# shangzhouye/stereo-visual-slam

Hardware: AMD Instinct MI355X
Metric: stereo keyframes/sec (ORB+match+tri+local-BA), KITTI-00 1241x376 (higher is better)
Workload: dtype u8+f64

## Files before the change

stereo-visual-slam_amd/csrc/api.hip:

```cpp
#include <stdarg.h>
#include <stdlib.h>

#include <algorithm>
#include <cmath>
#include <cfloat>
#include <vector>

#include "se3_device.h"
#include "vslam_internal.h"

#include <mutex>

namespace vslam {

static thread_local char g_err[512] = "";
void set_error(const char* fmt, ...) {
    va_list ap;
    va_start(ap, fmt);
    vsnprintf(g_err, sizeof(g_err), fmt, ap);
    va_end(ap);
}

struct Prof {
    struct Rec { const char* name; int launches; hipEvent_t e0, e1; };
    bool on = false;
    std::vector<Rec> recs, open;
    std::vector<hipEvent_t> pool;
    hipEvent_t get() {
        if (!pool.empty()) { hipEvent_t e = pool.back(); pool.pop_back(); return e; }
        hipEvent_t e = nullptr;
        (void)hipEventCreate(&e);
        return e;
    }
};
static thread_local Prof* g_prof = nullptr;
static hipEvent_t g_prof_origin[16] = {nullptr};
static std::mutex g_prof_origin_mu;
Prof* prof_current() { return g_prof; }
void prof_set_current(Prof* p) { g_prof = p; }
void prof_begin(hipStream_t s, const char* name, int launches) {
    Prof* p = g_prof;
    if (!p || !p->on) return;
    Prof::Rec r{name, launches, p->get(), p->get()};
    (void)hipEventRecord(r.e0, s);
    p->open.push_back(r);
}
void prof_end(hipStream_t s) {
    Prof* p = g_prof;
    if (!p || !p->on || p->open.empty()) return;
    Prof::Rec r = p->open.back();
    p->open.pop_back();
    (void)hipEventRecord(r.e1, s);
    p->recs.push_back(r);
}
#define VS_ENTER(c)                                                                         \
    do {                                                                                    \
        VS_HIP(hipSetDevice((c)->device));                                                  \
        prof_set_current(((c)->prof && (c)->prof->on) ? (c)->prof : nullptr);               \
    } while (0)

int DevBuf::reserve(size_t need, hipStream_t stream) {
    if (bytes >= need) return VSLAM_OK;
    VS_HIP(hipStreamSynchronize(stream));
    release();
    const size_t want = std::max(need, min_bytes);
    if (hipMalloc((void**)&p, want) != hipSuccess) { p = nullptr; set_error("%s hipMalloc(%zu) failed", name, want); return VSLAM_ERR_HIP; }
    bytes = want; *acct += want;
    return VSLAM_OK;
}
void DevBuf::release() {
    if (p) { (void)hipFree(p); *acct -= bytes; }
    p = nullptr; bytes = 0;
}

struct Arena : Layout {
    struct Upload { void* d; const void* h; size_t bytes; };
    std::vector<Upload> uploads;
    explicit Arena(uint8_t* b = nullptr) : Layout(b) {}
    template <typename T> T* in(const T* h, size_t n) { T* d = take<T>(n); if (base) uploads.push_back({d, h, n * sizeof(T)}); return d; }
};
template <typename F>
static int arena_stage(Ctx* c, F&& layout) {
    Arena a;
    if (int rc = carve(c->stage, c->stream, a, layout)) return rc;
    for (const Arena::Upload& u : a.uploads) VS_HIP(hipMemcpyAsync(u.d, u.h, u.bytes, hipMemcpyHostToDevice, c->stream));
    return VSLAM_OK;
}

static CamParams cam_of(const Ctx* c) {
    CamParams cam;
    cam.fx = c->p.cam[0]; cam.fy = c->p.cam[1]; cam.cx = c->p.cam[2]; cam.cy = c->p.cam[3]; cam.b = c->p.cam[4];
    cam.dmin = c->p.depth_min; cam.dmax = c->p.depth_max; cam.drel = c->p.depth_reliable; cam.row_tol = c->p.stereo_row_tol;
    return cam;
}

template <typename T>
static int dev_alloc(Ctx* c, T** p, size_t n) {
    VS_HIP(hipMalloc((void**)p, n * sizeof(T)));
    c->dev_bytes += n * sizeof(T);
    return VSLAM_OK;
}

struct TuneKey { const char* name; const char* env; int Tuning::*field; int lo, hi; };
static const TuneKey kTuneKeys[] = {
    {"orb_fuse_min", "VSLAM_ORB_FUSE_MIN", &Tuning::orb_fuse_min, 0, 1 << 30},
    {"sgbm_fuse_min", "VSLAM_SGBM_FUSE_MIN", &Tuning::sgbm_fuse_min, 0, 1 << 30},
    {"sgbm_fwd_min", "VSLAM_SGBM_FWD_MIN", &Tuning::sgbm_fwd_min, 0, 1 << 30},
    {"sgbm_fw_rows", "VSLAM_SGBM_FW_ROWS", &Tuning::sgbm_fw_rows, 32, 64},
    {"pose_only_window", "VSLAM_POSE_ONLY_WINDOW", &Tuning::pose_only_window, 0, 1},
    {"ba_resident", "VSLAM_BA_RESIDENT", &Tuning::ba_resident, 0, 1},
    {"pnp_window", "VSLAM_PNP_WINDOW", &Tuning::pnp_window, 0, 1},
    {"ba_adaptive", "VSLAM_BA_ADAPTIVE", &Tuning::ba_adaptive, 0, 1},
    {"ba_lanes", "VSLAM_BA_LANES", &Tuning::ba_lanes, 256, 512},
    {"track_rule", "VSLAM_TRACK_RULE", &Tuning::track_rule, 0, 1},
};
static int tune_set(Tuning& t, const TuneKey& k, long v) {
    if (v == -1) { t.*(k.field) = -1; return VSLAM_OK; }
    if (v < k.lo || v > k.hi || (k.field == &Tuning::sgbm_fw_rows && v != 32 && v != 64) || (k.field == &Tuning::ba_lanes && v != 256 && v != 512)) {
        set_error("tuning value %s = %ld out of range (%d..%d%s, or -1 = default)", k.name, v, k.lo, k.hi, k.field == &Tuning::sgbm_fw_rows ? ", 32 or 64" : "");
        return VSLAM_ERR_ARG;
    }
    t.*(k.field) = (int)v;
    return VSLAM_OK;
}
static int tune_from_env(Tuning& t) {
    for (const TuneKey& k : kTuneKeys) {
        const char* e = getenv(k.env);
        if (!e || !*e) continue;
        char* end = nullptr;
        const long v = strtol(e, &end, 10);
        if (end == e || *end != 0) { set_error("environment variable %s = \"%s\" is not an integer", k.env, e); return VSLAM_ERR_ARG; }
        int rc = tune_set(t, k, v);
        if (rc) return rc;
    }
    return VSLAM_OK;
}

static int orb_status_check(Ctx* c, int B) {
    std::vector<int32_t> st(B);
    VS_HIP(hipMemcpyAsync(st.data(), c->orb.d_status, sizeof(int32_t) * B, hipMemcpyDeviceToHost, c->stream));
    VS_HIP(hipStreamSynchronize(c->stream));
    for (int b = 0; b < B; ++b)
        if (st[b]) { set_error("ORB capacity exceeded on image %d (status bits 0x%x)", b, st[b]); return VSLAM_ERR_CAPACITY; }
    return VSLAM_OK;
}

constexpr int kOrbFuseMinDefault = 96;
static int orb_fuse_min(const Ctx* c) { return c->tune.orb_fuse_min >= 0 ? c->tune.orb_fuse_min : kOrbFuseMinDefault; }

static int orb_pipeline(Ctx* c, const uint8_t* d_imgs, size_t img_bytes, int pitch, int B, int anms_num, int regroup, bool describe,
                        vslam_keypoint* d_kps, uint8_t* d_desc, int32_t* d_count) {
    if (B <= 0) return VSLAM_OK;
    if (B > c->p.max_batch) { set_error("batch %d exceeds context max_batch %d", B, c->p.max_batch); return VSLAM_ERR_ARG; }
    int rc;
    const bool fused = describe && B >= orb_fuse_min(c);
    if (fused) {
        if ((rc = launch_orb_pyrblur(c->plan, c->tab, d_imgs, img_bytes, pitch, B, c->orb.d_pyr, c->orb.d_blur, c->p.fast_threshold, c->orb.d_corners,
                                     c->orb.d_corner_cnt, c->orb.d_status, c->stream))) return rc;
    } else {
        if ((rc = launch_orb_pyramid(c->plan, c->tab, d_imgs, img_bytes, pitch, B, c->orb.d_pyr, c->stream))) return rc;
        if ((rc = launch_orb_fast(c->plan, d_imgs, img_bytes, pitch, B, c->orb.d_pyr, c->p.fast_threshold, c->orb.d_corners,
                                  c->orb.d_corner_cnt, c->orb.d_status, c->stream))) return rc;
    }
    if ((rc = launch_orb_select(c->plan, d_imgs, img_bytes, pitch, B, c->orb.d_pyr, c->orb.d_corners, c->orb.d_corner_cnt, c->orb.d_sel,
                                c->orb.d_sel_cnt, c->orb.d_status, c->stream))) return rc;
    if ((rc = launch_orb_anms(c->plan, B, c->orb.d_sel, c->orb.d_sel_cnt, c->plan.sel_cap, anms_num, regroup, d_kps, nullptr, c->orb.d_order, c->p.kp_capacity,
                              d_count, c->orb.d_status, c->orb.d_rad, c->stream))) return rc;
    if ((rc = launch_orb_orient(c->plan, d_imgs, img_bytes, pitch, B, c->orb.d_pyr, d_kps, c->orb.d_cs, c->orb.d_order, c->p.kp_capacity, d_count, c->stream))) return rc;
    if (describe) {
        if (!fused && (rc = launch_orb_blur(c->plan, d_imgs, img_bytes, pitch, B, c->orb.d_pyr, c->orb.d_blur, c->stream))) return rc;
        if ((rc = launch_orb_describe(c->plan, d_imgs, img_bytes, pitch, B, c->orb.d_pyr, c->orb.d_blur, d_kps, c->orb.d_cs, c->orb.d_order, c->p.kp_capacity, d_count,
                                      d_desc, c->stream))) return rc;
    }
    if (getenv("VSLAM_ORB_PROFILE")) orb_debug_dump(c->stream);
    return VSLAM_OK;
}

static int check_img(Ctx* c, const void* img, int w, int h, int stride) {
    if (!c || !img) { set_error("null context or image"); return VSLAM_ERR_ARG; }
    if (w != c->p.img_w || h != c->p.img_h || stride < w) { set_error("image %dx%d (stride %d) does not match the context's %dx%d", w, h, stride, c->p.img_w, c->p.img_h); return VSLAM_ERR_ARG; }
    return VSLAM_OK;
}

}

using namespace vslam;

extern "C" {

void vslam_default_params(vslam_params* p) {
    if (!p) return;
    memset(p, 0, sizeof(*p));
    p->img_w = 1241; p->img_h = 376; p->max_batch = 1;
    p->orb_nfeatures = 3000; p->anms_num = 500; p->fast_threshold = 20; p->kp_capacity = 4096;
    p->cam[0] = 718.856; p->cam[1] = 718.856; p->cam[2] = 607.1928; p->cam[3] = 185.2157; p->cam[4] = 0.573;
    p->depth_min = 10; p->depth_max = 400; p->depth_reliable = 40;
    p->match_ratio = 2.0; p->match_gap_thr = 30.0; p->huber_delta = 5.991; p->pnp_reproj_thr = 4.0; p->stereo_row_tol = 2.0;
    p->struct_size = (int32_t)sizeof(vslam_params); p->abi_version = VSLAM_ABI_VERSION;
}

const char* vslam_last_error(void) { return g_err; }
const char* vslam_version(void) { return "vslam_hip 0.3 (gfx950, ABI 3)"; }
int vslam_abi_version(void) { return VSLAM_ABI_VERSION; }
const char* vslam_kernel_names(void) {
    return "orb_resize_kernel orb_pyrblur_kernel orb_fast_kernel orb_select_kernel orb_anms_kernel orb_orient_kernel orb_blur_kernel orb_describe_kernel "
           "match_train_nearest_kernel match_finalize_kernel sgbm_prefilter_kernel sgbm_down_kernel sgbm_forward_kernel sgbm_hsum_kernel sgbm_vsum_kernel sgbm_path_kernel "
           "sgbm_wta_kernel sgbm_lrcheck_kernel sgbm_median3_kernel sgbm_ccl_rows_kernel sgbm_ccl_union_kernel sgbm_ccl_count_kernel "
           "sgbm_ccl_apply_kernel sgbm_ccl_kernels triangulate_kernel find3d_disparity_kernel gather_uv_kernel build_pnp_inputs_kernel lm_window_kernel pose_only_wave_kernel "
           "lm_window_kernel<pnp> pnp_wave_kernel pnp_inlier_kernel pnp_epnp_kernels epnp_front_kernel epnp_jacobi_kernel epnp_back_kernel pnp_count_inliers_kernel hbm_copy_probe_kernel "
           "pnp_ransac_subsets_kernel pnp_ransac_count_kernel pnp_ransac_select_kernel "
           "build_windows_kernels track_init_kernel track_pose_chain_kernel track_link_kernel track_chain_kernel window_count_kernel window_scan_kernel window_rank_kernel window_emit_kernel "
           "track_ends_kernel kf_band_kernel kf_set_kernel kf_sliding_kernel kf_gate_kernel map_pnp_inputs_kernels track_map_inputs_kernel "
           "match_train_nearest_sel_kernel track_features_kernel";
}

int vslam_create(const vslam_params* p, int device, void* stream, vslam_ctx** out) {
    if (!p || !out) { set_error("null argument"); return VSLAM_ERR_ARG; }
    *out = nullptr;
    if (p->struct_size != (int32_t)sizeof(vslam_params) || p->abi_version != VSLAM_ABI_VERSION) {
        set_error("vslam_params from a different ABI (struct_size %d / abi_version %d, library has %d / %d): rebuild the caller against include/vslam_hip.h and "
                  "fill the struct with vslam_default_params", p->struct_size, p->abi_version, (int)sizeof(vslam_params), VSLAM_ABI_VERSION);
        return VSLAM_ERR_ARG;
    }
    int ndev = 0;
    if (hipGetDeviceCount(&ndev) != hipSuccess || ndev <= 0) { set_error("no HIP device visible (libvslam_hip has no CPU path)"); return VSLAM_ERR_NO_DEVICE; }
    if (device < 0 || device >= ndev) { set_error("device %d out of range (0..%d)", device, ndev - 1); return VSLAM_ERR_ARG; }
    if (p->max_batch <= 0 || p->kp_capacity < 64 || p->kp_capacity > kMaxRows || p->orb_nfeatures <= 0) { set_error("bad params (max_batch>0, 64<=kp_capacity<=%d)", kMaxRows); return VSLAM_ERR_ARG; }
    VS_HIP(hipSetDevice(device));
    Ctx* c = new Ctx();
    c->p = *p; c->device = device;
    c->lm.tune = &c->tune;
    { int rc_t = tune_from_env(c->tune); if (rc_t) { delete c; return rc_t; } }
    if (stream) { c->stream = (hipStream_t)stream; c->own_stream = false; }
    else {
        if (hipStreamCreateWithFlags(&c->stream, hipStreamNonBlocking) != hipSuccess) { set_error("hipStreamCreate failed"); delete c; return VSLAM_ERR_HIP; }
        c->own_stream = true;
    }
    if (getenv("VSLAM_ORB_PROFILE")) orb_debug_enable();
    int rc = orb_plan_init(&c->plan, p->img_w, p->img_h, p->orb_nfeatures, p->kp_capacity);
    if (rc == VSLAM_OK) { rc = orb_tables_init(&c->plan, &c->tab); c->dev_bytes += c->tab.bytes; }
    const size_t B = (size_t)p->max_batch;
    if (rc == VSLAM_OK) rc = dev_alloc(c, &c->orb.d_pyr, B * c->plan.pyr_bytes);
    if (rc == VSLAM_OK) rc = dev_alloc(c, &c->orb.d_corners, B * c->plan.corner_total);
    if (rc == VSLAM_OK) rc = dev_alloc(c, &c->orb.d_corner_cnt, B * kNLevels);
    if (rc == VSLAM_OK) rc = dev_alloc(c, &c->orb.d_sel, B * kNLevels * c->plan.sel_cap);
    if (rc == VSLAM_OK) rc = dev_alloc(c, &c->orb.d_sel_cnt, B * kNLevels);
    if (rc == VSLAM_OK) rc = dev_alloc(c, &c->orb.d_status, B);
    if (rc == VSLAM_OK) rc = dev_alloc(c, &c->orb.d_blur, B * c->plan.blur_bytes);
    if (rc == VSLAM_OK) rc = dev_alloc(c, &c->orb.d_cs, B * (size_t)p->kp_capacity);
    if (rc == VSLAM_OK) rc = dev_alloc(c, &c->orb.d_order, B * (size_t)p->kp_capacity);
    if (rc == VSLAM_OK) rc = dev_alloc(c, &c->orb.d_rad, B * (size_t)kMaxRows);
    if (rc == VSLAM_OK) rc = dev_alloc(c, &c->match.d_train_best, B * kMaxRows);
    if (rc != VSLAM_OK) { vslam_destroy(reinterpret_cast<vslam_ctx*>(c)); return rc; }
    *out = reinterpret_cast<vslam_ctx*>(c);
    return VSLAM_OK;
// ... 1046 lines not shown
```

stereo-visual-slam_amd/csrc/orb_kernels.hip:

```cpp
#include "vslam_internal.h"

#include <math.h>

#include <vector>

#include "orb_pattern.inc"

namespace vslam {

constexpr int kBlurTileH = 64;

__device__ __constant__ signed char c_pattern[256 * 4];

__device__ long long* g_orb_dbg = nullptr;
constexpr int kDbgRows = 8192;
#define OPH_INIT() long long* dbg__ = g_orb_dbg ? g_orb_dbg + 64 * (size_t)((blockIdx.x + 977u * blockIdx.y) % kDbgRows) : nullptr; long long tph__ = dbg__ ? clock64() : 0
#define OPH_ON() (dbg__ != nullptr)
#define OPH(slot) do { if (dbg__ && threadIdx.x == 0) { const long long t1__ = clock64(); dbg__[(slot) & 63] += t1__ - tph__; tph__ = t1__; } } while (0)
static long long* g_orb_dbg_host = nullptr;
void orb_debug_enable() {
    if (g_orb_dbg_host) return;
    hipMalloc((void**)&g_orb_dbg_host, sizeof(long long) * 64 * kDbgRows);
    hipMemset(g_orb_dbg_host, 0, sizeof(long long) * 64 * kDbgRows);
    hipMemcpyToSymbol(HIP_SYMBOL(g_orb_dbg), &g_orb_dbg_host, sizeof(g_orb_dbg_host));
}
void orb_debug_dump(hipStream_t stream) {
    if (!g_orb_dbg_host) return;
    hipStreamSynchronize(stream);
    static long long hall[64 * kDbgRows];
    hipMemcpy(hall, g_orb_dbg_host, sizeof(hall), hipMemcpyDeviceToHost);
    hipMemset(g_orb_dbg_host, 0, sizeof(hall));
    long long h[64] = {0};
    for (int r = 0; r < kDbgRows; ++r) for (int i = 0; i < 64; ++i) h[i] += hall[64 * r + i];
    static const char* names[64] = {"sel: hist+cut", "sel: harris", "sel: radix select", "sel: compact+sort", "sel: angle+out", nullptr, nullptr, nullptr,
                                    "desc: patch load", "desc: row blur", "desc: col blur", "desc: sincos+tests", nullptr, nullptr, nullptr, nullptr,
                                    "fast: tile load", "fast: corner test", "fast: score", "fast: nms+append", nullptr, nullptr, nullptr, nullptr,
                                    "anms: gather+sort", "anms: radii", "anms: radius sort", "anms: compact+regroup+out", nullptr, nullptr, nullptr, nullptr,
                                    "pyrfast: tile load", "pyrfast: resize", "pyrfast: blur", "pyrfast: edge columns", "pyrfast: pre-test", "pyrfast: queue pushes", "pyrfast: scores",
                                    "pyrfast: flush + barrier", "pyrfast: nms", "pyrfast: output"};
    for (int i = 0; i < 64; ++i) if (names[i] && h[i]) fprintf(stderr, "  [orb profile] %-28s %14lld block-cycles (sum over blocks)\n", names[i], h[i]);
}
static bool g_pattern_uploaded[16] = {false};

constexpr int kStCornerOverflow = 1, kStCandOverflow = 2, kStSelOverflow = 4, kStAnmsOverflow = 8, kStOutOverflow = 16;

__device__ inline int reflect101(int p, int len) {
    if (len == 1) return 0;
    while (p < 0 || p >= len) p = p < 0 ? -p : 2 * (len - 1) - p;
    return p;
}

struct LevelView {
    const uint8_t* ptr;
    int w, h, pitch;
};

struct LevelTable {
    int w[kNLevels], h[kNLevels], pitch[kNLevels], pyr_off[kNLevels];
    float scale[kNLevels];
    int nfeat[kNLevels];
    int corner_cap[kNLevels], corner_off[kNLevels];
    int tiles_x[kNLevels], tile_off[kNLevels + 1];
};

__device__ inline LevelView level_view(const LevelTable& T, int l, const uint8_t* img, int pitch0, const uint8_t* pyr) {
    LevelView v;
    v.w = T.w[l]; v.h = T.h[l];
    if (l == 0) { v.ptr = img; v.pitch = pitch0; }
    else { v.ptr = pyr + T.pyr_off[l]; v.pitch = T.pitch[l]; }
    return v;
}

__device__ inline uint4 shl_bytes_128(uint4 v, int s) {
    for (int t = 0; t < (s >> 2); ++t) { v.w = v.z; v.z = v.y; v.y = v.x; v.x = 0; }
    const uint32_t b = (uint32_t)s & 3u;
    if (b) {
        v.w = __builtin_amdgcn_alignbyte(v.w, v.z, 4u - b); v.z = __builtin_amdgcn_alignbyte(v.z, v.y, 4u - b);
        v.y = __builtin_amdgcn_alignbyte(v.y, v.x, 4u - b); v.x <<= 8u * b;
    }
    return v;
}
__device__ inline uint4 shr_bytes_128(uint4 v, int s) {
    for (int t = 0; t < (s >> 2); ++t) { v.x = v.y; v.y = v.z; v.z = v.w; v.w = 0; }
    const uint32_t b = (uint32_t)s & 3u;
    if (b) {
        v.x = __builtin_amdgcn_alignbyte(v.y, v.x, b); v.y = __builtin_amdgcn_alignbyte(v.z, v.y, b);
// ... 1543 lines not shown
            keep = v > s[-1] && v > s[1] && v > s[-kPfScPitch - 1] && v > s[-kPfScPitch] && v > s[-kPfScPitch + 1] && v > s[kPfScPitch - 1] &&
                   v > s[kPfScPitch] && v > s[kPfScPitch + 1];
            rec = (uint32_t)(ox + c - 4) | (uint32_t)(oy + R - 4) << 12 | (uint32_t)v << 24;
        }
        const unsigned long long bal = __ballot(keep);
        if (bal) {
            int base = 0;
            if (lane == 0) base = atomicAdd(&s_ocount, __popcll(bal));
            base = __builtin_amdgcn_readfirstlane(base);
            if (keep) outq[base + mbcnt64(bal)] = rec;
        }
    };
    if (!s_dense) {
        const int nc = s_ccount;
        for (int q = 64 * wave; q < nc; q += NT) nms_emit(q + lane < nc, q + lane < nc ? s_cq[q + lane] : 0);
    } else {
        for (int i = threadIdx.x; i < 64 * kBlurTileH; i += NT) {
            const int r = i >> 6, d = i & 63;
            uint32_t m = reinterpret_cast<const uint32_t*>(sc + (r + 1) * kPfScPitch)[1 + d];
            if (r <= vy_lo || r >= vy_hi) m = 0;
#pragma unroll 1
            for (int k = 0; k < 4; ++k) {
                const int tcx = 4 * d + k;
                const bool is = ((m >> (8 * k)) & 0xFFu) != 0 && tcx > vx_lo && tcx < vx_hi;
                if (__ballot(is)) nms_emit(is, (r + 4) << 9 | (tcx + 4));
            }
        }
    }
    __syncthreads();
    OPH(40);
    const int no = s_ocount;
    if (no > 0) {
        if (threadIdx.x == 0) s_obase = atomicAdd(a.corner_cnt + b * kNLevels, no);
        __syncthreads();
        uint32_t* corners = a.corners + (size_t)b * a.corner_img_stride;
        const int cap = a.corner_cap, base = s_obase;
        for (int q = threadIdx.x; q < no; q += NT) {
            if (base + q < cap) corners[base + q] = outq[q];
            else atomicOr(&a.status[b], kStCornerOverflow);
        }
    }
    OPH(41);
}

int launch_orb_pyrblur(const OrbPlan& plan, const OrbTables& tab, const uint8_t* d_imgs, size_t img_bytes, int pitch, int B, uint8_t* d_pyr,
                       uint8_t* d_blur, int fast_thr, uint32_t* d_corners, int32_t* d_corner_cnt, int32_t* d_status, hipStream_t stream) {
    if (d_corners) {
        VS_HIP(hipMemsetAsync(d_corner_cnt, 0, sizeof(int32_t) * B * kNLevels, stream));
        VS_HIP(hipMemsetAsync(d_status, 0, sizeof(int32_t) * B, stream));
    }
    ProfScope prof__(stream, "orb_pyrblur_kernel", kNLevels);
    for (int l = 0; l < kNLevels; ++l) {
        const OrbLevel& S = plan.lv[l];
        PyrBlurArgs a;
        memset(&a, 0, sizeof(a));
        a.src_base = l == 0 ? d_imgs : d_pyr + S.pyr_off;
        a.src_img_stride = l == 0 ? img_bytes : (size_t)plan.pyr_bytes;
        a.spitch = l == 0 ? pitch : ((S.w + 63) & ~63);
        a.sw = S.w; a.sh = S.h;
        a.blur_base = d_blur + plan.blur_off[l]; a.blur_img_stride = (size_t)plan.blur_bytes; a.bpitch = (S.w + 63) & ~63;
        a.tiles_x = (S.w + kBlurTileW - 1) / kBlurTileW;
        const int tiles_y = (S.h + kBlurTileH - 1) / kBlurTileH;
        if (l + 1 < kNLevels) {
            const OrbLevel& D = plan.lv[l + 1];
            a.dst_base = d_pyr + D.pyr_off; a.dst_img_stride = (size_t)plan.pyr_bytes; a.dpitch = (D.w + 63) & ~63; a.dw = D.w; a.dh = D.h;
            a.xofs = tab.d_xofs + tab.x_off[l + 1]; a.ialpha = tab.d_ialpha + 2 * tab.x_off[l + 1];
            a.yofs = tab.d_yofs + tab.y_off[l + 1]; a.ibeta = tab.d_ibeta + 2 * tab.y_off[l + 1];
            a.tile_dx = tab.d_tile_dx + tab.tdx_off[l]; a.tile_dy = tab.d_tile_dy + tab.tdy_off[l];
        }
        if (d_corners) {
            a.corners = d_corners + S.corner_off; a.corner_img_stride = (size_t)plan.corner_total; a.corner_cap = S.corner_cap;
            a.corner_cnt = d_corner_cnt + l; a.status = d_status; a.thr = fast_thr; a.level = l;
        }
        hipLaunchKernelGGL(orb_pyrblur_kernel<kPfWaves>, dim3(a.tiles_x * tiles_y, B), dim3(64 * kPfWaves), 0, stream, a);
    }
    VS_HIP(hipGetLastError());
    return VSLAM_OK;
}

constexpr int kDescWaves = 4;
constexpr int kDescR = 19, kDescRows = 2 * kDescR + 1, kDescPitch = 40;

constexpr int kDescBlocksPerImage = 48;
constexpr int kDescPatchIters = (kDescRows * (kDescPitch / 4) + 63) / 64;
__global__ __launch_bounds__(kDescWaves * 64) void orb_describe_kernel(BlurTable T, LevelTable LT, const uint8_t* __restrict__ d_imgs,
                                                                      size_t img_bytes, int pitch0, const uint8_t* __restrict__ d_pyr,
                                                                      size_t pyr_bytes, const uint8_t* __restrict__ d_blur, size_t blur_bytes,
                                                                      const vslam_keypoint* __restrict__ d_kps, const float2* __restrict__ d_cs,
                                                                      const int32_t* __restrict__ d_order, int kp_capacity,
                                                                      const int32_t* __restrict__ d_count, uint8_t* __restrict__ d_desc, int nb, int B) {
    int b, bx;
    if (!xcd_image_block(nb, B, b, bx)) return;
    const int wave = __builtin_amdgcn_readfirstlane(threadIdx.x >> 6), lane = threadIdx.x & 63;
    const int nwaves = nb * kDescWaves;
    const int n = min(d_count[b], kp_capacity);
    const int i0 = bx * kDescWaves + wave;
    if (i0 >= n) return;
    int slots;
    {
        const int i = i0 + lane * nwaves;
        slots = i < n ? (d_order ? min(max(d_order[(size_t)b * kp_capacity + i], 0), n - 1) : i) : -1;
    }
    const int nvisit = min((n - i0 + nwaves - 1) / nwaves, 64);
    int visit = 0;
    int j = __builtin_amdgcn_readlane(slots, 0);
    const vslam_keypoint* kps = d_kps + (size_t)b * kp_capacity;
    const float2* css = d_cs + (size_t)b * kp_capacity;
    __shared__ __attribute__((aligned(16))) uint8_t patch[kDescWaves][kDescRows * kDescPitch];
    uint8_t* pl = patch[wave];
    float px0[4], py0[4], px1[4], py1[4];
#pragma unroll
    for (int k = 0; k < 4; ++k) {
        const signed char* q = &c_pattern[(4 * lane + k) * 4];
        px0[k] = (float)q[0]; py0[k] = (float)q[1]; px1[k] = (float)q[2]; py1[k] = (float)q[3];
    }
    int prow[kDescPatchIters], pcol[kDescPatchIters];
#pragma unroll
    for (int it = 0; it < kDescPatchIters; ++it) {
        const int i = lane + 64 * it;
        prow[it] = i / (kDescPitch / 4); pcol[it] = 4 * (i - prow[it] * (kDescPitch / 4));
    }
    struct Geo { int cx, cy, l, W, H, bpitch; bool inside; const uint8_t* blur; };
    auto geometry = [&](const vslam_keypoint& kp) -> Geo {
        Geo g;
        g.l = __builtin_amdgcn_readfirstlane(min(max(kp.octave, 0), kNLevels - 1));
        g.W = T.w[g.l]; g.H = T.h[g.l]; g.bpitch = T.pitch[g.l];
        g.blur = d_blur + (size_t)b * blur_bytes + T.blur_off[g.l];
        const float inv_scale = __fdiv_rn(1.f, LT.scale[g.l]);
        g.cx = __builtin_amdgcn_readfirstlane(__float2int_rn(__fmul_rn(kp.x, inv_scale)));
        g.cy = __builtin_amdgcn_readfirstlane(__float2int_rn(__fmul_rn(kp.y, inv_scale)));
        g.inside = g.cx - kDescR >= 0 && g.cx + kDescR + 1 < g.W && g.cy - kDescR >= 0 && g.cy + kDescR < g.H;
        return g;
    };
    auto patch_fetch = [&](const Geo& g, uint32_t (&pv)[kDescPatchIters]) {
        if (!g.inside) return;
        const uint8_t* org = g.blur + (size_t)(g.cy - kDescR) * g.bpitch + (g.cx - kDescR);
#pragma unroll
        for (int it = 0; it < kDescPatchIters; ++it)
            if (prow[it] < kDescRows) __builtin_memcpy(&pv[it], org + (__umul24((uint32_t)prow[it], (uint32_t)g.bpitch) + (uint32_t)pcol[it]), 4);
    };
    vslam_keypoint kp = kps[j];
    float2 cs = css[j];
    Geo g = geometry(kp);
    uint32_t pv[kDescPatchIters];
    patch_fetch(g, pv);
    auto slot_of = [&](int v) -> int { return v < nvisit ? __builtin_amdgcn_readlane(slots, v) : -1; };
    int j1 = slot_of(1);
    vslam_keypoint kp1 = kps[max(j1, 0)];
    float2 cs1 = css[max(j1, 0)];
    for (;;) {
        if (g.inside) {
#pragma unroll
            for (int it = 0; it < kDescPatchIters; ++it)
                if (prow[it] < kDescRows) *reinterpret_cast<uint32_t*>(pl + prow[it] * kDescPitch + pcol[it]) = pv[it];
        }
        const Geo g1 = geometry(kp1);
        uint32_t pv1[kDescPatchIters];
        if (j1 >= 0) patch_fetch(g1, pv1);
        const int j2 = slot_of(visit + 2);
        const vslam_keypoint kp2 = kps[max(j2, 0)];
        const float2 cs2 = css[max(j2, 0)];
        __builtin_amdgcn_wave_barrier();
        const float ca = cs.x, sa = cs.y;
        int nib = 0;
        if (g.inside) {
#pragma unroll
            for (int k = 0; k < 4; ++k) {
                const int ix0 = __float2int_rn(__fsub_rn(__fmul_rn(px0[k], ca), __fmul_rn(py0[k], sa)));
                const int iy0 = __float2int_rn(__fadd_rn(__fmul_rn(px0[k], sa), __fmul_rn(py0[k], ca)));
                const int ix1 = __float2int_rn(__fsub_rn(__fmul_rn(px1[k], ca), __fmul_rn(py1[k], sa)));
                const int iy1 = __float2int_rn(__fadd_rn(__fmul_rn(px1[k], sa), __fmul_rn(py1[k], ca)));
                const int t0 = pl[(iy0 + kDescR) * kDescPitch + ix0 + kDescR], t1 = pl[(iy1 + kDescR) * kDescPitch + ix1 + kDescR];
                nib |= (t0 < t1) << k;
            }
        } else {
            const uint8_t* rawp = g.l == 0 ? d_imgs + (size_t)b * img_bytes : d_pyr + (size_t)b * pyr_bytes + T.pyr_off[g.l];
            const int rpitch = g.l == 0 ? pitch0 : T.pitch[g.l];
            auto sample = [&](int ix, int iy) -> int {
                const int x = g.cx + ix, y = g.cy + iy;
                if (x >= 0 && x < g.W && y >= 0 && y < g.H) return g.blur[(size_t)y * g.bpitch + x];
                return rawp[(size_t)reflect101(y, g.H) * rpitch + reflect101(x, g.W)];
            };
#pragma unroll
            for (int k = 0; k < 4; ++k) {
                const int ix0 = __float2int_rn(__fsub_rn(__fmul_rn(px0[k], ca), __fmul_rn(py0[k], sa)));
                const int iy0 = __float2int_rn(__fadd_rn(__fmul_rn(px0[k], sa), __fmul_rn(py0[k], ca)));
                const int ix1 = __float2int_rn(__fsub_rn(__fmul_rn(px1[k], ca), __fmul_rn(py1[k], sa)));
                const int iy1 = __float2int_rn(__fadd_rn(__fmul_rn(px1[k], sa), __fmul_rn(py1[k], ca)));
                nib |= (sample(ix0, iy0) < sample(ix1, iy1)) << k;
            }
        }
        const int hi = __shfl_down(nib, 1);
        if ((lane & 1) == 0) d_desc[((size_t)b * kp_capacity + j) * 32 + (lane >> 1)] = (uint8_t)(nib | (hi << 4));
        if (j1 < 0) break;
        __builtin_amdgcn_wave_barrier();
        ++visit;
        j = j1; j1 = j2; g = g1; cs = cs1; kp1 = kp2; cs1 = cs2;
#pragma unroll
        for (int it = 0; it < kDescPatchIters; ++it) pv[it] = pv1[it];
    }
}

int launch_orb_describe(const OrbPlan& plan, const uint8_t* d_imgs, size_t img_bytes, int pitch, int B, const uint8_t* d_pyr,
                        const uint8_t* d_blur, const vslam_keypoint* d_kps, const float2* d_cs, const int32_t* d_order, int kp_capacity, const int32_t* d_count,
                        uint8_t* d_desc, hipStream_t stream) {
    BlurTable T;
    fill_blur_table(plan, &T);
    LevelTable LT;
    fill_level_table(plan, &LT);
    const int max_kp = min(kp_capacity, kMaxRows);
    const int blocks = min(kDescBlocksPerImage, (max_kp + kDescWaves - 1) / kDescWaves);
    ProfScope prof__(stream, "orb_describe_kernel");
    hipLaunchKernelGGL(orb_describe_kernel, dim3(blocks * ((B + 7) / 8 * 8)), dim3(kDescWaves * 64), 0, stream, T, LT, d_imgs,
                       img_bytes, pitch, d_pyr, (size_t)plan.pyr_bytes, d_blur, (size_t)plan.blur_bytes, d_kps, d_cs, d_order, kp_capacity, d_count, d_desc, blocks, B);
    VS_HIP(hipGetLastError());
    return VSLAM_OK;
}

}
```

stereo-visual-slam_amd/csrc/vslam_internal.h:

```cpp
#pragma once
#include <hip/hip_runtime.h>
#include <stdint.h>
#include <stdio.h>
#include <string.h>

#include "../../include/vslam_hip.h"

namespace vslam {

void set_error(const char* fmt, ...);

#define VS_HIP(call)                                                                              \
    do {                                                                                          \
        hipError_t e__ = (call);                                                                  \
        if (e__ != hipSuccess) {                                                                  \
            ::vslam::set_error("%s:%d %s -> %s", __FILE__, __LINE__, #call, hipGetErrorString(e__)); \
            return VSLAM_ERR_HIP;                                                                 \
        }                                                                                         \
    } while (0)

struct Prof;
Prof* prof_current();
void prof_set_current(Prof* p);
void prof_begin(hipStream_t s, const char* name, int launches);
// ... 37 lines not shown
template <typename F>
int carve(DevBuf& buf, hipStream_t stream, F&& layout) { Layout a; return carve(buf, stream, a, layout); }

constexpr int kWave = 64;
constexpr int kNLevels = VSLAM_ORB_NLEVELS;
constexpr int kEdge = 31;
constexpr int kMaxRows = 4096;

struct OrbLevel {
    int w, h;
    float scale;
    int nfeat;
    int pyr_off;
    int corner_cap;
    int corner_off;
    int tiles_x, tiles_y, tile_off;
    int tab_off;
};

struct OrbPlan {
    OrbLevel lv[kNLevels];
    int w, h;
    int pyr_bytes;
    int corner_total;
    int total_tiles;
    int sel_cap;
    int blur_off[kNLevels];
    int blur_bytes;
};

struct Ctx;

struct OrbTables {
    int* d_xofs;
    short* d_ialpha;
    int* d_yofs;
    short* d_ibeta;
    int x_off[kNLevels], y_off[kNLevels];
    int* d_tile_dx;
    int* d_tile_dy;
    int tdx_off[kNLevels], tdy_off[kNLevels];
    size_t bytes;
};

void orb_debug_enable();
void orb_debug_dump(hipStream_t stream);
int orb_plan_init(OrbPlan* plan, int w, int h, int nfeatures, int kp_capacity);
int orb_tables_init(const OrbPlan* plan, OrbTables* t);
void orb_tables_free(OrbTables* t);

struct OrbBuffers {
    uint8_t* d_pyr;
    uint32_t* d_corners;
    int32_t* d_corner_cnt;
    vslam_keypoint* d_sel;
    int32_t* d_sel_cnt;
    int32_t* d_status;
    vslam_keypoint* d_det;
    uint8_t* d_blur;
    float2* d_cs;
    int32_t* d_order;
    double* d_rad;
};

int launch_orb_pyramid(const OrbPlan& plan, const OrbTables& tab, const uint8_t* d_imgs, size_t img_bytes, int pitch,
                       int B, uint8_t* d_pyr, hipStream_t stream);
int launch_orb_pyrblur(const OrbPlan& plan, const OrbTables& tab, const uint8_t* d_imgs, size_t img_bytes, int pitch, int B, uint8_t* d_pyr,
                       uint8_t* d_blur, int fast_thr, uint32_t* d_corners, int32_t* d_corner_cnt, int32_t* d_status, hipStream_t stream);
int launch_orb_fast(const OrbPlan& plan, const uint8_t* d_imgs, size_t img_bytes, int pitch, int B, const uint8_t* d_pyr,
                    int fast_thr, uint32_t* d_corners, int32_t* d_corner_cnt, int32_t* d_status, hipStream_t stream);
int launch_orb_select(const OrbPlan& plan, const uint8_t* d_imgs, size_t img_bytes, int pitch, int B, const uint8_t* d_pyr,
                      const uint32_t* d_corners, const int32_t* d_corner_cnt, vslam_keypoint* d_sel, int32_t* d_sel_cnt,
                      int32_t* d_status, hipStream_t stream);
int launch_orb_anms(const OrbPlan& plan, int B, const vslam_keypoint* d_sel, const int32_t* d_sel_cnt, int sel_cap,
                    int anms_num, int regroup, vslam_keypoint* d_kps, float2* d_cs, int32_t* d_order, int kp_capacity, int32_t* d_count, int32_t* d_status,
                    double* d_rad, hipStream_t stream);
int launch_anms_flat(int B, const vslam_keypoint* d_in, const int32_t* d_nin, int in_capacity, int anms_num, int regroup,
                     int img_w, int img_h, vslam_keypoint* d_kps, float2* d_cs, int32_t* d_order, int kp_capacity, int32_t* d_count, int32_t* d_status,
                     double* d_rad, hipStream_t stream);
int launch_orb_blur(const OrbPlan& plan, const uint8_t* d_imgs, size_t img_bytes, int pitch, int B, const uint8_t* d_pyr, uint8_t* d_blur,
                    hipStream_t stream);
int launch_orb_orient(const OrbPlan& plan, const uint8_t* d_imgs, size_t img_bytes, int pitch, int B, const uint8_t* d_pyr, vslam_keypoint* d_kps,
                      float2* d_cs, const int32_t* d_order, int kp_capacity, const int32_t* d_count, hipStream_t stream);
int launch_orb_describe(const OrbPlan& plan, const uint8_t* d_imgs, size_t img_bytes, int pitch, int B, const uint8_t* d_pyr,
                        const uint8_t* d_blur, const vslam_keypoint* d_kps, const float2* d_cs, const int32_t* d_order, int kp_capacity, const int32_t* d_count,
                        uint8_t* d_desc, hipStream_t stream);

struct MatchBuffers {
    uint32_t* d_train_best;
};
int launch_match(const uint8_t* d_q, size_t q_stride, const int32_t* d_nq, const uint8_t* d_t, size_t t_stride,
                 const int32_t* d_nt, const double* d_gap, int gate, double ratio, double gap_thr, int B, int max_rows,
                 uint32_t* d_train_best, vslam_dmatch* d_out, int out_capacity, int32_t* d_nout, hipStream_t stream,
                 const int32_t* d_qsel = nullptr, int sel_cap = 0, const int32_t* d_nqsel = nullptr);

struct CamParams { double fx, fy, cx, cy, b, dmin, dmax, drel, row_tol; };
int launch_find3d_disparity(const vslam_keypoint* d_kps, int n, const float* d_disp, int w, int h, int dstride,
                            const double* d_T, CamParams cam, float* d_xyz, uint8_t* d_valid, uint8_t* d_rel, hipStream_t stream);
int launch_find3d_disparity_batch(const vslam_keypoint* d_kps, const int32_t* d_n, int kp_capacity, int B, const float* d_disp, int w, int h,
                                  const double* d_T, CamParams cam, float* d_xyz, uint8_t* d_valid, uint8_t* d_rel, hipStream_t stream);
int launch_triangulate(const float* d_uvL, const float* d_uvR, const int32_t* d_n, int capacity, int B, const double* d_T,
                       CamParams cam, float* d_xyz, uint8_t* d_valid, uint8_t* d_rel, hipStream_t stream);
int launch_build_pnp_inputs(const vslam_dmatch* d_m, const int32_t* d_nm, int match_capacity, const vslam_dmatch* d_lr,
                            const int32_t* d_nlr, int lr_capacity, const float* d_xyz_lr, const uint8_t* d_valid_lr,
                            const vslam_keypoint* d_kpsT, int kp_capacity, int B, int32_t* d_kp2lr, float* d_xyz_out, float* d_uv_out,
                            int32_t* d_nout, int out_capacity, hipStream_t stream);
int launch_gather_uv(const vslam_keypoint* d_kpsQ, const vslam_keypoint* d_kpsT, int kp_capacity, const vslam_dmatch* d_m,
                     const int32_t* d_nm, int match_capacity, int B, float* d_uvQ, float* d_uvT, hipStream_t stream);

int launch_hbm_copy_probe(const void* src, void* dst, size_t bytes, int variant, hipStream_t stream);
int hbm_copy_probe_variants();
const char* hbm_copy_probe_name(int variant);

struct LmWindowArgs {
    int n_windows, n_kf;
    const int32_t* n_kf_w;
    const int32_t* lm_off;
    const int32_t* edge_off;
    double* T;
    float* xyz;
    const uint8_t* reliable;
    uint8_t* lm_inlier;
    const int32_t* kf_idx;
    const int32_t* lm_idx;
    const float* uv;
    double* chi2;
    vslam_lm_stats* stats;
    double* P;
    double* Ptrial;
    double* Hll;
    double* bl;
    double* Dinv;
    double* lin;
    int32_t* lm_ptr;
    int32_t* kf_ptr;
    int32_t* kf_edges;
    int32_t* pair_ptr;
    int32_t* pair_hits;
    int32_t hit_capacity_per_edge;
    double K[4];
    double huber_delta;
    double* chi2_thr;
    size_t total_lm, total_edge;
};
struct Tuning {
    int orb_fuse_min = -1;
    int sgbm_fuse_min = -1;
    int sgbm_fwd_min = -1;
    int sgbm_fw_rows = -1;
    int pose_only_window = -1;
    int pnp_window = -1;
    int ba_lanes = -1;
    int ba_resident = -1;
    int track_rule = -1;
    int ba_adaptive = -1;
};
constexpr int kSgbmTicketPools = 8;
constexpr int kSgbmErrorWord = kSgbmTicketPools;
int launch_sgbm(const Tuning& tune, const uint8_t* d_left, const uint8_t* d_right, size_t img_bytes, int pitch, int w, int h, int B, float* d_disp_f32,
                int16_t* d_disp_i16, int16_t* d_disp_raw, DevBuf& scratch, hipStream_t stream);

struct LmScratch {
    DevBuf buf, cyc;
    int32_t* status = nullptr; int status_n = 0;
    int32_t* passes = nullptr;
    const Tuning* tune = nullptr;
    bool lds_opt_in = false;
    bool rs_opt_in = false;
    int rs_dyn_bytes = -1, rs_full_bytes = 0, rs_cu_count = 0;
    int32_t* defer = nullptr;
    bool defer_valid = false;
    explicit LmScratch(size_t* acct) : buf("LM scratch", acct), cyc("LM clock buffer", acct) {}
};
struct RsLaunch {
    LmWindowArgs a;
    void* uv_s; int32_t* epos; double* tab; double* xin; double* Pbak; double* Dc; double* blc;
    int32_t* status; int32_t* passes; int32_t* defer; const int32_t* order; long long* dbg;
    int dyn_bytes, full_bytes, cu_count;
    int schedule, adaptive, iters, update_poses, update_lms, dense_to_general;
    int want_chi2;
    int lanes;
    bool opt_in_done;
};
void rs_query_device(int device, LmScratch& s);
int launch_ba_resident(const RsLaunch& L, hipStream_t stream);
int launch_lm_windows(const LmWindowArgs& a, int schedule, int mode, int iters, int update_poses, int update_lms, LmScratch* scratch,
                      hipStream_t stream);
size_t lm_hits_per_edge();
int lm_fetch_status(const LmScratch* scratch, int n_windows, int32_t* h_status, hipStream_t stream);
int lm_fetch_passes(const LmScratch* scratch, int n_windows, int32_t* h_passes, hipStream_t stream);
int lm_fetch_deferred(const LmScratch* scratch, int n_windows, int32_t* h_defer, hipStream_t stream);

struct PnpArgs {
    const float* xyz; const float* uv; const int32_t* n; int capacity; int B;
    double* T; int iters; double K[4]; double huber_delta; double reproj_thr;
    uint8_t* inlier; int32_t* n_inliers; vslam_lm_stats* stats;
    int n_hint;
};
int launch_pnp(const PnpArgs& a, LmScratch* scratch, hipStream_t stream);
int launch_edge_jacobians(int n, const float* d_xyz, const float* d_uv, const double* d_T, const double K[4], double delta, double* d_err, double* d_Jp, double* d_Jl,
                          double* d_chi2, double* d_hw, hipStream_t stream);
size_t pnp_epnp_ws_bytes(int H);
int launch_pnp_epnp(const float* d_hx, const float* d_hu, int H, const double K[4], double* d_Rt, double* d_T, int32_t* d_ok, uint8_t* ws, hipStream_t stream);
int launch_pnp_count_inliers(const float* d_xyz, const float* d_uv, int n, const double* d_Rt, const int32_t* d_ok, int hyp0, int n_hyp, const double K[4],
                             double reproj_thr, int32_t* d_counts, uint8_t* d_mask, hipStream_t stream);

int launch_pnp_ransac_batch(const float* d_xyz, const float* d_uv, const int32_t* d_n, int capacity, int B, int H, const double K[4], double reproj_err,
                            double confidence, DevBuf& scratch, double* d_T, uint8_t* d_inlier, int32_t* d_n_inl, int32_t* d_iters, hipStream_t stream);
struct KfPolicy { int policy; double near_dist; int32_t* kf_frame; int32_t* evicted; bool gate = false; const int32_t* num_inliers = nullptr; int32_t* frame_state = nullptr;
                  const double* G = nullptr; const int32_t* in_of_match = nullptr; const int32_t* state_in = nullptr; };
int launch_build_windows(const vslam_tracks_in& in, int n_kf, int lm_capacity, int edge_capacity, const double K4[4], double reproj_thr, int track_rule, DevBuf& scratch,
                         int32_t* d_lm_off, int32_t* d_edge_off, int32_t* d_n_kf, double* d_T, float* d_xyz_out, uint8_t* d_rel_out, uint8_t* d_inl_out,
                         int32_t* d_kf_out, int32_t* d_lm_out, float* d_uv_out, int32_t* d_status, const KfPolicy& kp, hipStream_t stream);
int launch_chain_poses(int n_frames, const double* d_T_rel, double* d_G, hipStream_t stream);
int launch_gate_states(int n_frames, const double* d_T, int absolute, const int32_t* d_num_inliers, int32_t* d_state, hipStream_t stream);
struct MapRequery { const uint8_t* d_desc; size_t desc_stride; int32_t* d_feat; int32_t* d_nfeat; vslam_dmatch* d_f2f_out; int32_t* d_nf2f_out;
                    double ratio, gap_thr; uint32_t* d_train_best; };
int launch_map_pnp_inputs(const vslam_tracks_in& in, const double* d_G, const int32_t* d_in_of_match_prev, const int32_t* d_state, const double K4[4],
                          double reproj_thr, int track_rule, DevBuf& scratch, float* d_xyz_out, float* d_uv_out, int32_t* d_n_out, int32_t* d_in_of_match,
                          int out_capacity, int32_t* d_status, hipStream_t stream, const MapRequery* rq = nullptr);

struct Ctx {
    vslam_params p;
    int device;
    hipStream_t stream;
    bool own_stream;
    size_t dev_bytes;
    OrbPlan plan;
    OrbTables tab;
// ... 15 lines not shown
```

Before: 63240.

## Fuse ORB orientation computation into the describe kernel

Adds a templated describe kernel that computes intensity-centroid orientation per keypoint inside each wave, using packed dot4 moments and shuffle reductions. The rotation is then fed straight into the BRIEF descriptor loop, replacing the separate orient launch and its cos/sin buffer round trip. The patch fetch is also restructured into six-row trips, with the SGPR budget constrained. This saves a kernel launch and global traffic, at the cost of extra register pressure and serial moment work before describing starts.

Measured after the change: 63610 (median of 6 runs). Within noise of the previous version (+0.6%).

```diff
diff --git a/stereo-visual-slam_amd/csrc/api.hip b/stereo-visual-slam_amd/csrc/api.hip
--- a/stereo-visual-slam_amd/csrc/api.hip
+++ b/stereo-visual-slam_amd/csrc/api.hip
@@ -104,6 +104,7 @@
 struct TuneKey { const char* name; const char* env; int Tuning::*field; int lo, hi; };
 static const TuneKey kTuneKeys[] = {
     {"orb_fuse_min", "VSLAM_ORB_FUSE_MIN", &Tuning::orb_fuse_min, 0, 1 << 30},
+    {"orb_orient_fuse", "VSLAM_ORB_ORIENT_FUSE", &Tuning::orb_orient_fuse, 0, 1},
     {"sgbm_fuse_min", "VSLAM_SGBM_FUSE_MIN", &Tuning::sgbm_fuse_min, 0, 1 << 30},
     {"sgbm_fwd_min", "VSLAM_SGBM_FWD_MIN", &Tuning::sgbm_fwd_min, 0, 1 << 30},
     {"sgbm_fw_rows", "VSLAM_SGBM_FW_ROWS", &Tuning::sgbm_fw_rows, 32, 64},
@@ -166,11 +167,16 @@
                                 c->orb.d_sel_cnt, c->orb.d_status, c->stream))) return rc;
     if ((rc = launch_orb_anms(c->plan, B, c->orb.d_sel, c->orb.d_sel_cnt, c->plan.sel_cap, anms_num, regroup, d_kps, nullptr, c->orb.d_order, c->p.kp_capacity,
                               d_count, c->orb.d_status, c->orb.d_rad, c->stream))) return rc;
-    if ((rc = launch_orb_orient(c->plan, d_imgs, img_bytes, pitch, B, c->orb.d_pyr, d_kps, c->orb.d_cs, c->orb.d_order, c->p.kp_capacity, d_count, c->stream))) return rc;
+    const bool orient_fused = describe && c->tune.orb_orient_fuse != 0;
+    if (!orient_fused &&
+        (rc = launch_orb_orient(c->plan, d_imgs, img_bytes, pitch, B, c->orb.d_pyr, d_kps, c->orb.d_cs, c->orb.d_order, c->p.kp_capacity, d_count, c->stream))) return rc;
     if (describe) {
         if (!fused && (rc = launch_orb_blur(c->plan, d_imgs, img_bytes, pitch, B, c->orb.d_pyr, c->orb.d_blur, c->stream))) return rc;
-        if ((rc = launch_orb_describe(c->plan, d_imgs, img_bytes, pitch, B, c->orb.d_pyr, c->orb.d_blur, d_kps, c->orb.d_cs, c->orb.d_order, c->p.kp_capacity, d_count,
-                                      d_desc, c->stream))) return rc;
+        if (orient_fused)
+            rc = launch_orb_orient_describe(c->plan, d_imgs, img_bytes, pitch, B, c->orb.d_pyr, c->orb.d_blur, d_kps, c->orb.d_order, c->p.kp_capacity, d_count, d_desc, c->stream);
+        else
+            rc = launch_orb_describe(c->plan, d_imgs, img_bytes, pitch, B, c->orb.d_pyr, c->orb.d_blur, d_kps, c->orb.d_cs, c->orb.d_order, c->p.kp_capacity, d_count, d_desc, c->stream);
+        if (rc) return rc;
     }
     if (getenv("VSLAM_ORB_PROFILE")) orb_debug_dump(c->stream);
     return VSLAM_OK;
diff --git a/stereo-visual-slam_amd/csrc/orb_kernels.hip b/stereo-visual-slam_amd/csrc/orb_kernels.hip
--- a/stereo-visual-slam_amd/csrc/orb_kernels.hip
+++ b/stereo-visual-slam_amd/csrc/orb_kernels.hip
@@ -2,6 +2,7 @@
 
 #include <math.h>
 
+#include <type_traits>
 #include <vector>
 
 #include "orb_pattern.inc"
@@ -1711,11 +1712,15 @@
 constexpr int kDescR = 19, kDescRows = 2 * kDescR + 1, kDescPitch = 40;
 
 constexpr int kDescBlocksPerImage = 48;
-constexpr int kDescPatchIters = (kDescRows * (kDescPitch / 4) + 63) / 64;
-__global__ __launch_bounds__(kDescWaves * 64) void orb_describe_kernel(BlurTable T, LevelTable LT, const uint8_t* __restrict__ d_imgs,
+constexpr int kDescFusedBlocksPerImage = 48;
+static_assert(64 * kDescWaves * kDescBlocksPerImage >= kMaxRows && 64 * kDescWaves * kDescFusedBlocksPerImage >= kMaxRows, "a lane holds one visit of its wave's walk");
+constexpr int kDescTripRows = 6, kDescPatchIters = (kDescRows + kDescTripRows - 1) / kDescTripRows;
+template <bool ORIENT>
+__global__ __launch_bounds__(kDescWaves * 64) __attribute__((amdgpu_num_sgpr(80))) void orb_describe_kernel(BlurTable T, LevelTable LT, const uint8_t* __restrict__ d_imgs,
                                                                       size_t img_bytes, int pitch0, const uint8_t* __restrict__ d_pyr,
                                                                       size_t pyr_bytes, const uint8_t* __restrict__ d_blur, size_t blur_bytes,
-                                                                      const vslam_keypoint* __restrict__ d_kps, const float2* __restrict__ d_cs,
+                                                                      typename std::conditional<ORIENT, vslam_keypoint, const vslam_keypoint>::type* __restrict__ d_kps,
+                                                                      const float2* __restrict__ d_cs,
                                                                       const int32_t* __restrict__ d_order, int kp_capacity,
                                                                       const int32_t* __restrict__ d_count, uint8_t* __restrict__ d_desc, int nb, int B) {
     int b, bx;
@@ -1733,62 +1738,163 @@
     const int nvisit = min((n - i0 + nwaves - 1) / nwaves, 64);
     int visit = 0;
     int j = __builtin_amdgcn_readlane(slots, 0);
-    const vslam_keypoint* kps = d_kps + (size_t)b * kp_capacity;
-    const float2* css = d_cs + (size_t)b * kp_capacity;
+    auto* kps = d_kps + (size_t)b * kp_capacity;
+    const float2* css = ORIENT ? nullptr : d_cs + (size_t)b * kp_capacity;
     __shared__ __attribute__((aligned(16))) uint8_t patch[kDescWaves][kDescRows * kDescPitch];
     uint8_t* pl = patch[wave];
-    float px0[4], py0[4], px1[4], py1[4];
-#pragma unroll
-    for (int k = 0; k < 4; ++k) {
-        const signed char* q = &c_pattern[(4 * lane + k) * 4];
-        px0[k] = (float)q[0]; py0[k] = (float)q[1]; px1[k] = (float)q[2]; py1[k] = (float)q[3];
-    }
-    int prow[kDescPatchIters], pcol[kDescPatchIters];
-#pragma unroll
-    for (int it = 0; it < kDescPatchIters; ++it) {
-        const int i = lane + 64 * it;
-        prow[it] = i / (kDescPitch / 4); pcol[it] = 4 * (i - prow[it] * (kDescPitch / 4));
-    }
+    int my_l = 0, my_x = 0, my_y = 0, my_ok = 0, my_m10 = 0, my_m01 = 0;
+    float my_ca = 1.f, my_sa = 0.f;
+    if constexpr (ORIENT) {
+        if (lane < nvisit) {
+            const vslam_keypoint kp = kps[slots];
+            my_l = min(max(kp.octave, 0), kNLevels - 1);
+            const float inv_scale = __fdiv_rn(1.f, LT.scale[my_l]);
+            my_x = __float2int_rn(__fmul_rn(kp.x, inv_scale)); my_y = __float2int_rn(__fmul_rn(kp.y, inv_scale));
+            my_ok = my_x >= 15 && my_y >= 15 && my_x + 16 <= LT.w[my_l] && my_y + 15 < LT.h[my_l];
+        }
+        const int ry = lane >> 3, cq = lane & 7;
+        uint32_t wt[4], wm[4]; int vs[4], rsel[4];
+        {
+            const uint4 a_ = *reinterpret_cast<const uint4*>(g_ic_lane.wt[lane]), m_ = *reinterpret_cast<const uint4*>(g_ic_lane.wm[lane]);
+            wt[0] = a_.x; wt[1] = a_.y; wt[2] = a_.z; wt[3] = a_.w; wm[0] = m_.x; wm[1] = m_.y; wm[2] = m_.z; wm[3] = m_.w;
+        }
+#pragma unroll
+        for (int s = 0; s < 4; ++s) {
+            const int v = -15 + ry + 8 * s;
+            vs[s] = v > 15 ? 0 : v; rsel[s] = min(ry + 8 * s, 30);
+        }
+        const uint8_t* img0 = d_imgs + (size_t)b * img_bytes;
+        const uint8_t* pyr0 = d_pyr + (size_t)b * pyr_bytes;
+        auto request = [&](int k0, uint32_t (&px)[4][4]) {
+#pragma unroll
+            for (int u = 0; u < 4; ++u) {
+                const bool ok = __builtin_amdgcn_readlane(my_ok, k0 + u) != 0;
+                const int x = ok ? __builtin_amdgcn_readlane(my_x, k0 + u) : 15, y = ok ? __builtin_amdgcn_readlane(my_y, k0 + u) : 15;
+                const int l = ok ? __builtin_amdgcn_readlane(my_l, k0 + u) : 0;
+                const uint8_t* base = l == 0 ? img0 : pyr0 + LT.pyr_off[l];
+                const int pitch = l == 0 ? pitch0 : LT.pitch[l];
+                const uint8_t* p0 = base + (size_t)(y - 15) * pitch + (x - 15);
+#pragma unroll
+                for (int s = 0; s < 4; ++s) __builtin_memcpy(&px[u][s], p0 + (uint32_t)(rsel[s] * pitch + 4 * cq), 4);
+            }
+        };
+        auto moments = [&](int k0, const uint32_t (&px)[4][4], int (&m)[8]) {
+#pragma unroll
+            for (int u = 0; u < 4; ++u) {
+                uint32_t tsum = 0, asum = 0; int m01 = 0;
+#pragma unroll
+                for (int s = 0; s < 4; ++s) {
+                    const uint32_t as = __builtin_amdgcn_udot4(px[u][s], wm[s], 0u, false);
+                    tsum = __builtin_amdgcn_udot4(px[u][s], wt[s], tsum, false);
+                    asum += as;
+                    m01 += vs[s] * (int)as;
+                }
+                const bool live = __builtin_amdgcn_readlane(my_ok, k0 + u) != 0;
+                m[2 * u] = live ? (int)tsum - 15 * (int)asum : 0;
+                m[2 * u + 1] = live ? m01 : 0;
+            }
+        };
+        auto reduce = [&](int k0, const int (&m)[8]) {
+            const bool h0 = (lane & 1) != 0, h1 = (lane & 2) != 0, h2 = (lane & 4) != 0;
+            int a4[4];
+#pragma unroll
+            for (int q = 0; q < 4; ++q) a4[q] = (h0 ? m[4 + q] : m[q]) + __shfl_xor(h0 ? m[q] : m[4 + q], 1);
+            int a2[2];
+#pragma unroll
+            for (int q = 0; q < 2; ++q) a2[q] = (h1 ? a4[2 + q] : a4[q]) + __shfl_xor(h1 ? a4[q] : a4[2 + q], 2);
+            int r = (h2 ? a2[1] : a2[0]) + __shfl_xor(h2 ? a2[0] : a2[1], 4);
+            for (int o = 8; o < 64; o <<= 1) r += __shfl_xor(r, o);
+#pragma unroll
+            for (int u = 0; u < 4; ++u) {
+                const int q = (u >> 1) | ((u & 1) << 1);
+                const int m10 = __builtin_amdgcn_readlane(r, q), m01 = __builtin_amdgcn_readlane(r, q + 4);
+                if (lane == k0 + u) { my_m10 = m10; my_m01 = m01; }
+            }
+        };
+        uint32_t pa[4][4];
+        request(0, pa);
+        for (int k0 = 0; k0 < nvisit; k0 += 4) {
+            int m[8];
+            moments(k0, pa, m);
+            if (k0 + 4 < nvisit) request(k0 + 4, pa);
+            reduce(k0, m);
+        }
+    }
+    const int prow0 = min(lane, 59) / (kDescPitch / 4), pcol = 4 * (min(lane, 59) - prow0 * (kDescPitch / 4));
+    static_assert(kDescTripRows * (kDescPitch / 4) <= 64 && kDescTripRows * kDescPatchIters >= kDescRows, "seven trips of six rows cover the patch");
+    const int plds = prow0 * kDescPitch + pcol;
     struct Geo { int cx, cy, l, W, H, bpitch; bool inside; const uint8_t* blur; };
-    auto geometry = [&](const vslam_keypoint& kp) -> Geo {
+    auto geometry_at = [&](int l, int cx, int cy) -> Geo {
         Geo g;
-        g.l = __builtin_amdgcn_readfirstlane(min(max(kp.octave, 0), kNLevels - 1));
+        g.l = l; g.cx = cx; g.cy = cy;
         g.W = T.w[g.l]; g.H = T.h[g.l]; g.bpitch = T.pitch[g.l];
         g.blur = d_blur + (size_t)b * blur_bytes + T.blur_off[g.l];
-        const float inv_scale = __fdiv_rn(1.f, LT.scale[g.l]);
-        g.cx = __builtin_amdgcn_readfirstlane(__float2int_rn(__fmul_rn(kp.x, inv_scale)));
-        g.cy = __builtin_amdgcn_readfirstlane(__float2int_rn(__fmul_rn(kp.y, inv_scale)));
         g.inside = g.cx - kDescR >= 0 && g.cx + kDescR + 1 < g.W && g.cy - kDescR >= 0 && g.cy + kDescR < g.H;
         return g;
+    };
+    auto geometry = [&](const vslam_keypoint& kp) -> Geo {
+        const int l = __builtin_amdgcn_readfirstlane(min(max(kp.octave, 0), kNLevels - 1));
+        const float inv_scale = __fdiv_rn(1.f, LT.scale[l]);
+        return geometry_at(l, __builtin_amdgcn_readfirstlane(__float2int_rn(__fmul_rn(kp.x, inv_scale))),
+                           __builtin_amdgcn_readfirstlane(__float2int_rn(__fmul_rn(kp.y, inv_scale))));
+    };
+    auto geometry_of_visit = [&](int v) -> Geo {
+        return geometry_at(__builtin_amdgcn_readlane(my_l, v), __builtin_amdgcn_readlane(my_x, v), __builtin_amdgcn_readlane(my_y, v));
+    };
+    auto rotation_of_visit = [&](int v) -> float2 {
+        return make_float2(__int_as_float(__builtin_amdgcn_readlane(__float_as_int(my_ca), v)), __int_as_float(__builtin_amdgcn_readlane(__float_as_int(my_sa), v)));
     };
     auto patch_fetch = [&](const Geo& g, uint32_t (&pv)[kDescPatchIters]) {
         if (!g.inside) return;
         const uint8_t* org = g.blur + (size_t)(g.cy - kDescR) * g.bpitch + (g.cx - kDescR);
+        const uint32_t voff = __umul24((uint32_t)prow0, (uint32_t)g.bpitch) + (uint32_t)pcol;
 #pragma unroll
         for (int it = 0; it < kDescPatchIters; ++it)
-            if (prow[it] < kDescRows) __builtin_memcpy(&pv[it], org + (__umul24((uint32_t)prow[it], (uint32_t)g.bpitch) + (uint32_t)pcol[it]), 4);
+            if (prow0 + kDescTripRows * it < kDescRows) __builtin_memcpy(&pv[it], org + (size_t)(kDescTripRows * it) * g.bpitch + voff, 4);
     };
-    vslam_keypoint kp = kps[j];
-    float2 cs = css[j];
-    Geo g = geometry(kp);
+    Geo g;
+    float2 cs;
     uint32_t pv[kDescPatchIters];
-    patch_fetch(g, pv);
+    if constexpr (ORIENT) {
+        g = geometry_of_visit(0);
+        patch_fetch(g, pv);
+        if (lane < nvisit) {
+            const float ang = fast_atan2_dev((float)my_m01, (float)my_m10);
+            kps[slots].angle = ang;
+            const float rad = __fmul_rn(ang, (float)(3.1415926535897932384626433832795 / 180.f));
+            my_ca = (float)cos((double)rad); my_sa = (float)sin((double)rad);
+        }
+        cs = rotation_of_visit(0);
+    } else {
+        cs = css[j];
+        g = geometry(kps[j]);
+        patch_fetch(g, pv);
+    }
+    float px0[4], py0[4], px1[4], py1[4];
+#pragma unroll
+    for (int k = 0; k < 4; ++k) {
+        const signed char* q = &c_pattern[(4 * lane + k) * 4];
+        px0[k] = (float)q[0]; py0[k] = (float)q[1]; px1[k] = (float)q[2]; py1[k] = (float)q[3];
+    }
     auto slot_of = [&](int v) -> int { return v < nvisit ? __builtin_amdgcn_readlane(slots, v) : -1; };
     int j1 = slot_of(1);
-    vslam_keypoint kp1 = kps[max(j1, 0)];
-    float2 cs1 = css[max(j1, 0)];
+    vslam_keypoint kp1{};
+    float2 cs1{};
+    if constexpr (!ORIENT) { kp1 = kps[max(j1, 0)]; cs1 = css[max(j1, 0)]; }
     for (;;) {
         if (g.inside) {
 #pragma unroll
             for (int it = 0; it < kDescPatchIters; ++it)
-                if (prow[it] < kDescRows) *reinterpret_cast<uint32_t*>(pl + prow[it] * kDescPitch + pcol[it]) = pv[it];
-        }
-        const Geo g1 = geometry(kp1);
+                if (prow0 + kDescTripRows * it < kDescRows) *reinterpret_cast<uint32_t*>(pl + plds + kDescTripRows * kDescPitch * it) = pv[it];
+        }
+        Geo g1;
+        if constexpr (ORIENT) g1 = geometry_of_visit(min(visit + 1, nvisit - 1)); else g1 = geometry(kp1);
         uint32_t pv1[kDescPatchIters];
         if (j1 >= 0) patch_fetch(g1, pv1);
         const int j2 = slot_of(visit + 2);
-        const vslam_keypoint kp2 = kps[max(j2, 0)];
-        const float2 cs2 = css[max(j2, 0)];
+        vslam_keypoint kp2{};
+        float2 cs2{};
+        if constexpr (!ORIENT) { kp2 = kps[max(j2, 0)]; cs2 = css[max(j2, 0)]; }
         __builtin_amdgcn_wave_barrier();
         const float ca = cs.x, sa = cs.y;
         int nib = 0;
@@ -1824,8 +1930,8 @@
         if (j1 < 0) break;
         __builtin_amdgcn_wave_barrier();
         ++visit;
-        j = j1; j1 = j2; g = g1; cs = cs1; kp1 = kp2; cs1 = cs2;
-#pragma unroll
+        j = j1; j1 = j2; g = g1;
+        if constexpr (ORIENT) cs = rotation_of_visit(visit); else { cs = cs1; kp1 = kp2; cs1 = cs2; }
         for (int it = 0; it < kDescPatchIters; ++it) pv[it] = pv1[it];
     }
 }
@@ -1840,10 +1946,27 @@
     const int max_kp = min(kp_capacity, kMaxRows);
     const int blocks = min(kDescBlocksPerImage, (max_kp + kDescWaves - 1) / kDescWaves);
     ProfScope prof__(stream, "orb_describe_kernel");
-    hipLaunchKernelGGL(orb_describe_kernel, dim3(blocks * ((B + 7) / 8 * 8)), dim3(kDescWaves * 64), 0, stream, T, LT, d_imgs,
+    hipLaunchKernelGGL(orb_describe_kernel<false>, dim3(blocks * ((B + 7) / 8 * 8)), dim3(kDescWaves * 64), 0, stream, T, LT, d_imgs,
                        img_bytes, pitch, d_pyr, (size_t)plan.pyr_bytes, d_blur, (size_t)plan.blur_bytes, d_kps, d_cs, d_order, kp_capacity, d_count, d_desc, blocks, B);
     VS_HIP(hipGetLastError());
     return VSLAM_OK;
 }
 
-}
+int launch_orb_orient_describe(const OrbPlan& plan, const uint8_t* d_imgs, size_t img_bytes, int pitch, int B, const uint8_t* d_pyr,
+                               const uint8_t* d_blur, vslam_keypoint* d_kps, const int32_t* d_order, int kp_capacity, const int32_t* d_count,
+                               uint8_t* d_desc, hipStream_t stream) {
+    BlurTable T;
+    fill_blur_table(plan, &T);
+    LevelTable LT;
+    fill_level_table(plan, &LT);
+    const int max_kp = min(kp_capacity, kMaxRows);
+    const int blocks = min(kDescFusedBlocksPerImage, (max_kp + kDescWaves - 1) / kDescWaves);
+    ProfScope prof__(stream, "orb_describe_kernel");
+    hipLaunchKernelGGL(orb_describe_kernel<true>, dim3(blocks * ((B + 7) / 8 * 8)), dim3(kDescWaves * 64), 0, stream, T, LT, d_imgs,
+                       img_bytes, pitch, d_pyr, (size_t)plan.pyr_bytes, d_blur, (size_t)plan.blur_bytes, d_kps, (const float2*)nullptr, d_order, kp_capacity, d_count, d_desc,
+                       blocks, B);
+    VS_HIP(hipGetLastError());
+    return VSLAM_OK;
+}
+
+}
diff --git a/stereo-visual-slam_amd/csrc/vslam_internal.h b/stereo-visual-slam_amd/csrc/vslam_internal.h
--- a/stereo-visual-slam_amd/csrc/vslam_internal.h
+++ b/stereo-visual-slam_amd/csrc/vslam_internal.h
@@ -143,6 +143,9 @@
                     hipStream_t stream);
 int launch_orb_orient(const OrbPlan& plan, const uint8_t* d_imgs, size_t img_bytes, int pitch, int B, const uint8_t* d_pyr, vslam_keypoint* d_kps,
                       float2* d_cs, const int32_t* d_order, int kp_capacity, const int32_t* d_count, hipStream_t stream);
+int launch_orb_orient_describe(const OrbPlan& plan, const uint8_t* d_imgs, size_t img_bytes, int pitch, int B, const uint8_t* d_pyr,
+                               const uint8_t* d_blur, vslam_keypoint* d_kps, const int32_t* d_order, int kp_capacity, const int32_t* d_count,
+                               uint8_t* d_desc, hipStream_t stream);
 int launch_orb_describe(const OrbPlan& plan, const uint8_t* d_imgs, size_t img_bytes, int pitch, int B, const uint8_t* d_pyr,
                         const uint8_t* d_blur, const vslam_keypoint* d_kps, const float2* d_cs, const int32_t* d_order, int kp_capacity, const int32_t* d_count,
                         uint8_t* d_desc, hipStream_t stream);
@@ -206,6 +209,7 @@
 };
 struct Tuning {
     int orb_fuse_min = -1;
+    int orb_orient_fuse = -1;
     int sgbm_fuse_min = -1;
     int sgbm_fwd_min = -1;
     int sgbm_fw_rows = -1;
```
